# arielgabizon/barretenberg

Measured on AMD Instinct MI355X. Metric: BN254 G1 MSM points/sec at n=2^20 (Fr NTT elems/sec in 'ntt'), higher is better.
Workload: dtype u32x9 (256-bit Montgomery, 29-bit limbs)

## Files before the change

barretenberg_amd/csrc/capi.hip:

```cpp
#include <hip/hip_runtime.h>

#include <algorithm>
#include <mutex>
#include <optional>
#include <stdarg.h>
#include <stdio.h>
#include <stdlib.h>
#include <string.h>
#include <time.h>
#include <atomic>
#include <condition_variable>
#include <exception>
#include <functional>
#include <thread>
#include <unordered_map>
#include <vector>

#include "bbgpu_internal.h"
#include "host_g1.hpp"
#include "host_g2.hpp"
#include "host_small.hpp"
#include "host_fallback.hpp"
#include "host_copy_pool.hpp"
#include "host_pairing.hpp"
#include "host_srs_check.hpp"
#include "host_srs_update.hpp"
#include "host_plonk_verify.hpp"
#include "multi_plan.hpp"
#include "poly.h"

namespace bbgpu {

static thread_local char g_err[512] = "";
void set_error(const char* fmt, ...)
{
    va_list ap;
    va_start(ap, fmt);
    vsnprintf(g_err, sizeof(g_err), fmt, ap);
    va_end(ap);
}

namespace {
enum FaultKind { F_ALLOC = 0, F_H2D = 1, F_D2H = 2, F_LAUNCH = 3, F_KINDS = 4 };
struct FaultState {
    std::mutex mu;
    std::atomic<int> armed_kind{ -1 };
    uint64_t fail_at = 0;
    std::atomic<uint64_t> calls[F_KINDS] = {};
    std::atomic<uint64_t> fired{ 0 }, absorbed{ 0 };
    std::unordered_map<void*, size_t> live;
    uint64_t live_bytes = 0;
    bool env_read = false;
};
FaultState& fault()
{
    static FaultState* f = new FaultState();
    return *f;
}
int fault_parse(const char* spec, int* kind, uint64_t* at)
{
    static const char* names[F_KINDS] = { "alloc", "h2d", "d2h", "launch" };
    if (!spec || !*spec) { *kind = -1; return 0; }
    for (int k = 0; k < F_KINDS; k++) {
        const size_t len = strlen(names[k]);
        if (!strncmp(spec, names[k], len) && spec[len] == ':') {
            char* end = nullptr;
            *at = strtoull(spec + len + 1, &end, 0);
            if (end == spec + len + 1 || *end) return -1;
            *kind = k;
            return 0;
        }
    }
    return -1;
}
int fault_set(const char* spec)
{
    FaultState& F = fault();
    int kind = -1;
    uint64_t at = 0;
    if (fault_parse(spec, &kind, &at)) return -1;
    std::lock_guard<std::mutex> lk(F.mu);
    F.env_read = true;
    for (auto& c : F.calls) c.store(0);
    F.fired.store(0);
    F.absorbed.store(0);
    F.fail_at = at;
    F.armed_kind.store(kind);
    return 0;
}
bool fault_hit(FaultKind kind)
{
    FaultState& F = fault();
    if (!F.env_read) {
        std::lock_guard<std::mutex> lk(F.mu);
        if (!F.env_read) {
            F.env_read = true;
            int k = -1;
            uint64_t at = 0;
            const char* e = getenv("BBGPU_FAIL_AT");
            if (e && fault_parse(e, &k, &at) == 0 && k >= 0) {
                F.fail_at = at;
                F.armed_kind.store(k);
            } else if (e && *e) {
                fprintf(stderr, "bbgpu: BBGPU_FAIL_AT=%s not understood (alloc:k | h2d:k | d2h:k | launch:k)\n", e);
            }
        }
    }
    const uint64_t n = F.calls[kind].fetch_add(1);
    if (F.armed_kind.load(std::memory_order_relaxed) != (int)kind) return false;
    std::lock_guard<std::mutex> lk(F.mu);
    if (F.armed_kind.load() != (int)kind || n != F.fail_at) return false;
// ... 28 lines not shown
        auto it = F.live.find(p);
        if (it != F.live.end()) {
            F.live_bytes -= it->second;
            F.live.erase(it);
        }
    }
    return hipFree(p);
}
hipError_t h2d_async(void* dst, const void* src, size_t bytes, hipStream_t st)
{
    if (fault_hit(F_H2D)) {
        set_error("hipMemcpyAsync(host to device, %zu bytes) -> %s [injected by BBGPU_FAIL_AT]", bytes, hipGetErrorString(hipErrorInvalidValue));
        return hipErrorInvalidValue;
    }
    return hipMemcpyAsync(dst, src, bytes, hipMemcpyHostToDevice, st);
}
hipError_t d2h_async(void* dst, const void* src, size_t bytes, hipStream_t st)
{
    if (fault_hit(F_D2H)) {
        set_error("hipMemcpyAsync(device to host, %zu bytes) -> %s [injected by BBGPU_FAIL_AT]", bytes, hipGetErrorString(hipErrorInvalidValue));
        return hipErrorInvalidValue;
    }
    return hipMemcpyAsync(dst, src, bytes, hipMemcpyDeviceToHost, st);
}
hipError_t launch_check()
{
    const hipError_t e = hipGetLastError();
    if (e != hipSuccess) return e;
    if (fault_hit(F_LAUNCH)) {
        set_error("kernel launch -> %s [injected by BBGPU_FAIL_AT]", hipGetErrorString(hipErrorLaunchFailure));
        return hipErrorLaunchFailure;
    }
    return hipSuccess;
}
void fault_absorbed() { fault().absorbed.fetch_add(1); }

namespace {

struct SrsEntry {
    const uint64_t* host_ptr;
    size_t n;
    uint32_t* d_srs;
    bool live;
    struct TabSeg {
        size_t first = 0, n = 0;
        uint32_t* d_tab = nullptr;
        uint32_t* d_tab_alloc = nullptr;
    };
    std::vector<TabSeg> segs;
    bool has_tab() const { return !segs.empty(); }
    int tab_c = 0, tab_W = 0, tab_wb = 0, tab_we = 0;
    std::vector<uint64_t> row_hash;
    bool auto_registered = false;
    uint64_t last_use = 0;
    size_t bytes = 0;
    bool handle_exposed = false;
    uint64_t check_phase = 0;
    bool stale_for_host = false;
    bool validate_full = false;
};

inline uint64_t hash_row(const uint64_t* row8)
{
    static const uint64_t M[8] = { 0x9e3779b97f4a7c15ULL, 0xbf58476d1ce4e5b9ULL, 0x94d049bb133111ebULL, 0xd6e8feb86659fd93ULL,
                                   0xca5a826395121157ULL, 0xff51afd7ed558ccdULL, 0xc4ceb9fe1a85ec53ULL, 0x2545f4914f6cdd1dULL };
    uint64_t h = 0;
    for (int i = 0; i < 8; i++) h += (row8[i] ^ M[(i + 3) & 7]) * M[i];
    h ^= h >> 31;
    return h * 0x9e3779b97f4a7c15ULL;
}

struct Context {
    bool ready = false;
    int device = 0;
    hipStream_t stream = nullptr;
    std::vector<SrsEntry> srs;
    static constexpr int NSLOT = 8;
    MsmSlot slot[NSLOT];
    int next_slot = 0;
    uint64_t* d_stage = nullptr;
    size_t stage_cap = 0;
    uint64_t* d_stage2 = nullptr;
    size_t stage2_cap = 0;
    uint64_t* d_scratch = nullptr;
    size_t scratch_cap = 0;
    uint64_t* d_small_tab = nullptr;
    size_t small_tab_cap = 0;
    uint64_t* d_srs_check = nullptr;
    size_t srs_check_cap = 0;
    uint64_t* d_verify = nullptr;
    size_t verify_cap = 0;
    int timing = 0;
    bool precompute = true;
    uint64_t use_clock = 0;
    size_t srs_cache_cap = (size_t)16 << 30;
    bool srs_validate_full = false;
    int host_msm_max = 24;
    int host_ntt_max = 16;
    bool host_env_read = false;
    int share_rank = 0, share_world = 1;
    int point_world = 1;
    hipEvent_t helper_dep[NSLOT] = {};
    hipEvent_t shared_done = nullptr;
    hipStream_t shared_last = nullptr;
    bool shared_used = false;
    poly::Scratch poly_scratch;
    uint64_t* d_poly_tmp = nullptr;
    size_t poly_tmp_cap = 0;
    MsmTiming last;
    static constexpr size_t HOST_CHUNK = (size_t)1 << 20;
    static constexpr int HOST_RING = 8;
    size_t host_chunk = HOST_CHUNK;
    void* h_stage[HOST_RING] = {};
    hipEvent_t h_stage_free[HOST_RING] = {};
    unsigned h_stage_next = 0;
    size_t host_stage_max = (size_t)8 << 20;
    bool stage_env_read = false;
    host::CopyPool copy_pool;
    AccRing acc_ring;
    size_t slice_of_n = 0;
    std::recursive_mutex own_mu;
};

std::recursive_mutex g_mu;
Context g_ctxs[BBGPU_MAX_CONTEXTS];
int g_num_ctx = 1;
thread_local int t_ctx = 0;
inline Context& ctx() { return g_ctxs[t_ctx]; }
inline std::recursive_mutex& ctx_lock() { return t_ctx == 0 ? g_mu : ctx().own_mu; }

#define CHK(x)                                                                                                         \
    do {                                                                                                               \
        hipError_t e_ = (x);                                                                                           \
        if (e_ != hipSuccess) {                                                                                        \
            set_error("%s:%d %s -> %s", __FILE__, __LINE__, #x, hipGetErrorString(e_));                                \
            return BBGPU_ERR_HIP;                                                                                      \
        }                                                                                                              \
    } while (0)

void read_host_env()
{
    if (!ctx().host_env_read) {
        ctx().host_env_read = true;
        if (const char* e = getenv("BBGPU_HOST_MSM_MAX")) ctx().host_msm_max = atoi(e);
        if (const char* e = getenv("BBGPU_HOST_NTT_MAX")) ctx().host_ntt_max = std::min(64, atoi(e));
    }
    if (ctx().stage_env_read) return;
    ctx().stage_env_read = true;
    if (const char* e = getenv("BBGPU_STAGE_MAX_BYTES")) ctx().host_stage_max = (size_t)strtoull(e, nullptr, 0);
    if (const char* e = getenv("BBGPU_STAGE_CHUNK_BYTES")) ctx().host_chunk = std::min(Context::HOST_CHUNK, std::max((size_t)64 << 10, (size_t)strtoull(e, nullptr, 0)));
}

int hip_device_count()
{
    static const int cnt = [] { int c = 0; return hipGetDeviceCount(&c) == hipSuccess ? c : 0; }();
    return cnt;
}

int ensure_init()
{
    std::lock_guard<std::recursive_mutex> lk(ctx_lock());
    if (ctx().ready) {
        static thread_local int bound_device = -1;
        if (bound_device != ctx().device) {
            CHK(hipSetDevice(ctx().device));
            bound_device = ctx().device;
        }
        return BBGPU_OK;
    }
    (void)setenv("GPU_MAX_HW_QUEUES", "16", 0);
    if (hip_device_count() == 0) {
        set_error("no HIP device available: the GPU entry points of libbbgpu have no CPU fallback");
        return BBGPU_ERR_HIP;
    }
    CHK(hipSetDevice(ctx().device));
    CHK(hipStreamCreateWithFlags(&ctx().stream, hipStreamNonBlocking));
    for (auto& sl : ctx().slot) {
        if (!sl.stream) CHK(hipStreamCreateWithFlags(&sl.stream, hipStreamNonBlocking));
        sl.acc_ring = &ctx().acc_ring;
    }
    CHK(hipEventCreateWithFlags(&ctx().shared_done, hipEventDisableTiming));
    ctx().shared_used = false;
    if (const char* e = getenv("BBGPU_SRS_CACHE_BYTES")) ctx().srs_cache_cap = (size_t)strtoull(e, nullptr, 0);
    if (const char* e = getenv("BBGPU_SRS_VALIDATE")) ctx().srs_validate_full = !strcmp(e, "full");
    ctx().ready = true;
    return BBGPU_OK;
}

int shared_begin(hipStream_t st)
{
    if (ctx().shared_used && ctx().shared_last != st) CHK(hipStreamWaitEvent(st, ctx().shared_done, 0));
    return BBGPU_OK;
}
int shared_end(hipStream_t st)
{
    CHK(hipEventRecord(ctx().shared_done, st));
    ctx().shared_last = st;
    ctx().shared_used = true;
    return BBGPU_OK;
}

int grow(uint64_t** buf, size_t* cap, size_t bytes)
{
    if (bytes <= *cap) return BBGPU_OK;
    if (*buf) (void)dev_free(*buf);
    *buf = nullptr;
    *cap = 0;
    CHK(dev_malloc((void**)buf, bytes));
    *cap = bytes;
    return BBGPU_OK;
}

}


int bind_calling_thread()
{
    return ensure_init();
}
static int host_stage_ensure()
{
    for (int k = 0; k < Context::HOST_RING; k++)
        if (!ctx().h_stage[k]) {
            CHK(hipHostMalloc(&ctx().h_stage[k], Context::HOST_CHUNK, hipHostMallocDefault));
            CHK(hipEventCreateWithFlags(&ctx().h_stage_free[k], hipEventDisableTiming));
        }
    return BBGPU_OK;
}
int host_to_device(void* d_dst, const void* h_src, size_t bytes, hipStream_t st)
{
    std::lock_guard<std::recursive_mutex> lk(ctx_lock());
    read_host_env();
    if (bytes == 0) return BBGPU_OK;
    if (bytes > ctx().host_stage_max) {
        CHK(h2d_async(d_dst, h_src, bytes, st));
        return BBGPU_OK;
    }
    if (int rc = host_stage_ensure()) return rc;
    const size_t CH = ctx().host_chunk;
    for (size_t off = 0; off < bytes; off += CH) {
        const size_t len = std::min(CH, bytes - off);
        const int k = (int)(ctx().h_stage_next++ % Context::HOST_RING);
        CHK(hipEventSynchronize(ctx().h_stage_free[k]));
        ctx().copy_pool.copy(ctx().h_stage[k], (const char*)h_src + off, len);
        CHK(h2d_async((char*)d_dst + off, ctx().h_stage[k], len, st));
        CHK(hipEventRecord(ctx().h_stage_free[k], st));
    }
    return BBGPU_OK;
}
int device_to_host_sync(void* h_dst, const void* d_src, size_t bytes, hipStream_t st, bool* touched)
{
    std::lock_guard<std::recursive_mutex> lk(ctx_lock());
    read_host_env();
    if (touched) *touched = false;
    if (bytes > ctx().host_stage_max) {
        CHK(d2h_async(h_dst, d_src, bytes, st));
        if (touched) *touched = true;
        CHK(hipStreamSynchronize(st));
        return BBGPU_OK;
    }
    if (int rc = host_stage_ensure()) return rc;
    const size_t CH = ctx().host_chunk;
    const size_t chunks = (bytes + CH - 1) / CH;
// ... 335 lines not shown
    const size_t stride = n / 14, phase = (size_t)((e.check_phase++ * 0x9e3779b97f4a7c15ULL) % stride);
    for (size_t k = 0; k < 14; k++)
        if (!same(phase + k * stride)) return false;
    return true;
}

bool contents_match_full(const SrsEntry& e, size_t off, const uint64_t* points, size_t n)
{
    if (e.row_hash.size() != e.n) return false;
    struct Job { const uint64_t* p; const uint64_t* h; std::atomic<int> bad; } job{ points, e.row_hash.data() + off, { 0 } };
    ctx().copy_pool.for_range(n, (size_t)1 << 14, [](void* c, size_t lo, size_t hi) {
        Job* j = static_cast<Job*>(c);
        uint64_t diff = 0;
        for (size_t i = lo; i < hi; i++) diff |= hash_row(j->p + i * 16) ^ j->h[i];
        if (diff) j->bad.store(1);
    }, &job);
    return job.bad.load() == 0;
}

struct FullCheckJob {
    const uint64_t* p = nullptr;
    const uint64_t* h = nullptr;
    std::atomic<int> bad{ 0 };
    bool posted = false;
};
void full_check_post(FullCheckJob& job, const SrsEntry& e, size_t off, const uint64_t* points, size_t n)
{
    job.p = points;
    job.h = e.row_hash.data() + off;
    job.bad.store(e.row_hash.size() != e.n ? 1 : 0);
    job.posted = true;
    if (job.bad.load()) return;
    ctx().copy_pool.post_range(n, [](void* c, size_t lo, size_t hi) {
        FullCheckJob* j = static_cast<FullCheckJob*>(c);
        uint64_t diff = 0;
        for (size_t i = lo; i < hi; i++) diff |= hash_row(j->p + i * 16) ^ j->h[i];
        if (diff) j->bad.store(1);
    }, &job);
}
bool full_check_join(FullCheckJob& job)
{
    ctx().copy_pool.join();
    job.posted = false;
    return job.bad.load() == 0;
}

int find_srs(const uint64_t* points, size_t n, size_t* offset, bool* deferred_full = nullptr)
{
    if (deferred_full) *deferred_full = false;
    for (size_t k = ctx().srs.size(); k-- > 0;) {
        SrsEntry& e = ctx().srs[k];
        if (!e.live || !e.host_ptr || e.stale_for_host) continue;
        const uint8_t* b = (const uint8_t*)e.host_ptr;
        const uint8_t* p = (const uint8_t*)points;
        if (p < b || p >= b + e.n * 128) continue;
        const size_t d = (size_t)(p - b);
        if (d % 128) continue;
        if (d / 128 + n > e.n) continue;
        if (!contents_match(e, d / 128, points, n) || (e.validate_full && !deferred_full && !contents_match_full(e, d / 128, points, n))) {
            if (trace_srs()) fprintf(stderr, "bbgpu srs: contents of %p (+%zu rows, n=%zu) differ from the resident copy\n", (const void*)e.host_ptr, d / 128, n);
            if (e.auto_registered) free_entry(e);
            else if (e.validate_full) e.stale_for_host = true;
            continue;
        }
        if (deferred_full) *deferred_full = e.validate_full;
        e.last_use = ++ctx().use_clock;
        *offset = d / 128;
        return (int)k;
    }
    return -1;
}

void srs_mark_stale(int idx)
{
    SrsEntry& e = ctx().srs[idx];
    if (trace_srs()) fprintf(stderr, "bbgpu srs: full check: contents of %p differ from the resident copy\n", (const void*)e.host_ptr);
    if (e.auto_registered) free_entry(e);
    else e.stale_for_host = true;
}

double now_ms() { timespec ts; clock_gettime(CLOCK_MONOTONIC, &ts); return ts.tv_sec * 1e3 + ts.tv_nsec * 1e-6; }

size_t largest_piece(const PointPiece* pc, int np) { size_t m = 0; for (int k = 0; k < np; k++) m = std::max(m, pc[k].len); return m; }
size_t collected_before(size_t p, int slots) { return p - std::min(p, (size_t)std::max(slots, 1) - 1); }
template <class Done> struct HostMsmPipeline {
    int sl[2] = { -1, -1 }, ns = 0;
    Done done;
    double ms_push = 0, ms_wait = 0;

    explicit HostMsmPipeline(Done d) : done(std::move(d)) {}
    HostMsmPipeline(const HostMsmPipeline&) = delete;
    ~HostMsmPipeline()
    {
        if (bg.posted) (void)full_check_join(bg);
        drain();
    }
    int open()
    {
        if (int rc = ensure_init()) return rc;
        if ((ns = free_slots(sl, 2)) == 0) {
            set_error("all %d MSM slots are in flight: call bbgpu_msm_g1_wait first", Context::NSLOT);
            return BBGPU_ERR_STATE;
        }
        reserve.emplace(sl, ns);
        return BBGPU_OK;
    }
    hipStream_t first_stream() const { return ctx().slot[sl[0]].stream; }
    int make_room() { return collected < collected_before(issued, ns) ? collect() : BBGPU_OK; }
    int push(const SrsEntry& e, size_t off, const uint64_t* scalars, size_t len, size_t stage_bytes, size_t tag, MsmTiming* timing)
    {
        if (int rc = make_room()) return rc;
        const size_t w = issued % (size_t)ns;
        MsmSlot& S = ctx().slot[sl[w]];
        const double t0 = tr ? now_ms() : 0;
        int rc = grow(stage[w], cap[w], stage_bytes);
        if (rc == BBGPU_OK) rc = host_to_device(*stage[w], scalars, len * 32, S.stream);
        if (rc == BBGPU_OK) rc = issue_ticket(sl[w], e, off, stage[w], 1, len, 0, entry_windows(e, len), S.stream);
        if (rc) { drain(); return rc; }
        if (tr) ms_push += now_ms() - t0;
        fl[w] = InFlight{ tag, timing };
        issued++;
        return BBGPU_OK;
    }
    void check_in_full(int idx, size_t off, const uint64_t* points, size_t n, bool background)
    {
        for (const auto& c : checks)
            if (c.idx == idx && c.off == off && c.n == n) return;
        if (background && checks.empty()) full_check_post(bg, ctx().srs[idx], off, points, n);
        checks.push_back(Check{ idx, off, points, n });
    }
    int finish(bool* stale)
    {
        for (size_t k = 0; k < checks.size(); k++) {
            const Check& c = checks[k];
            const bool same = (k == 0 && bg.posted) ? full_check_join(bg) : !ctx().srs[c.idx].live || contents_match_full(ctx().srs[c.idx], c.off, c.points, c.n);
            if (!same) {
                srs_mark_stale(c.idx);
                *stale = true;
            }
        }
        if (*stale) {
            drain();
            return BBGPU_OK;
        }
        while (collected < issued)
            if (int rc = collect()) return rc;
        return BBGPU_OK;
    }

private:
    struct InFlight { size_t tag; MsmTiming* timing; } fl[2] = {};
    size_t issued = 0, collected = 0;
    uint64_t** stage[2] = { &ctx().d_stage, &ctx().d_stage2 };
    size_t* cap[2] = { &ctx().stage_cap, &ctx().stage2_cap };
    std::optional<SlotReservation> reserve;
    struct Check { int idx; size_t off; const uint64_t* points; size_t n; };
    std::vector<Check> checks;
    FullCheckJob bg;
    const bool tr = trace_srs();

    int collect()
    {
        const size_t w = collected++ % (size_t)ns;
        const double t0 = tr ? now_ms() : 0;
        host::Xyzz sum;
        if (int rc = finish_ticket(sl[w], &sum, fl[w].timing)) { drain(); return rc; }
        done(fl[w].tag, sum);
        if (tr) ms_wait += now_ms() - t0;
        return BBGPU_OK;
    }
    void drain()
    {
        drain_tickets(sl, ns);
        collected = issued;
    }
};

template <class Once> int rerun_if_stale(Once once)
{
    bool stale = false;
    int rc = once(&stale);
    if (stale) rc = once(&stale);
    return rc;
}

int log2_exact(size_t n)
{
    if (n == 0 || (n & (n - 1))) return -1;
    int l = 0;
    while (((size_t)1 << l) < n) l++;
    return l;
}

int msm_host_ptrs_once(const uint64_t* scalars, const uint64_t* points, size_t n, host::Xyzz* out, bool plain, bool* stale);
int msm_host_ptrs_sum(const uint64_t* scalars, const uint64_t* points, size_t n, host::Xyzz* out, bool plain = false)
{
    return rerun_if_stale([&](bool* stale) { return msm_host_ptrs_once(scalars, points, n, out, plain, stale); });
}
int msm_host_ptrs(const uint64_t* scalars, const uint64_t* points, size_t n, uint64_t out[12], bool plain = false)
{
    host::Xyzz res;
    const int rc = msm_host_ptrs_sum(scalars, points, n, &res, plain);
    if (rc == BBGPU_OK) host::g1_to_normalised(res, out);
    return rc;
}
int msm_host_ptrs_once(const uint64_t* scalars, const uint64_t* points, size_t n, host::Xyzz* out, bool plain, bool* stale)
{
    *stale = false;
    if (n == 0) {
        *out = host::g1_infinity();
        return BBGPU_OK;
    }
    if (!scalars || !points) {
        set_error("null scalars/points");
        return BBGPU_ERR_ARG;
    }
    size_t off = 0;
    bool full_check = false;
    int idx = plain ? -1 : find_srs(points, n, &off, &full_check);
    read_host_env();
    if (idx < 0 && n <= (size_t)ctx().host_msm_max) {
        *out = host::msm_small(scalars, points, n, plain ? 8 : 16);
        return BBGPU_OK;
    }
    host::Xyzz res = host::g1_infinity();
    HostMsmPipeline P([&res](size_t, const host::Xyzz& part) { res = host::g1_add(res, part); });
    if (int rc = P.open()) return rc;
    if (full_check) P.check_in_full(idx, off, points, n, n * 32 > ctx().host_stage_max);
    SrsEntry transient{};
    const bool is_transient = idx < 0 && (plain || n < AUTO_REGISTER_MIN_POINTS);
    const bool tr = trace_srs();
    const double q0 = tr ? now_ms() : 0;
    const bool small_once = is_transient && n < AUTO_REGISTER_MIN_POINTS;
    if (idx < 0) {
        uint32_t* d = nullptr;
        int rc = BBGPU_OK;
        if (small_once) {
            if ((rc = grow(&ctx().d_small_tab, &ctx().small_tab_cap, AUTO_REGISTER_MIN_POINTS * (128 + 64))) != BBGPU_OK) return rc;
            uint32_t* d_raw = (uint32_t*)ctx().d_small_tab;
            d = d_raw + AUTO_REGISTER_MIN_POINTS * 32;
            rc = srs_upload_into(points, n, d_raw, d, P.first_stream(), plain ? 64 : 128);
        } else {
            rc = srs_upload(points, n, &d, ctx().stream, plain ? 64 : 128);
        }
        if (rc) return rc;
        if (is_transient) {
            transient.host_ptr = points;
            transient.n = n;
            transient.d_srs = d;
            transient.live = true;
        } else if ((idx = add_srs(points, n, d, true)) < 0) {
            return idx;
        }
        off = 0;
    }
    const SrsEntry& e = is_transient ? transient : ctx().srs[idx];
    static const size_t split_env = [] { const char* v = getenv("BBGPU_HOST_MSM_SPLIT"); return v ? (size_t)std::min(MAX_POINT_PIECES, std::max(1, atoi(v))) : (size_t)0; }();
    PointPiece pc[MAX_POINT_PIECES];
    int np = split_pieces(e, off, n, pc, MAX_POINT_PIECES);
    if (np < 0) return BBGPU_ERR_SIZE;
    if (np == 1) {
        const size_t parts = P.ns < 2 ? 1 : (split_env ? split_env : (n >= ((size_t)1 << 19) ? 2 : 1));
        const size_t base = parts == 2 ? ((n * 3 / 8) & ~(size_t)7) : n / parts;
        np = 0;
        for (size_t k = 0; k < parts; k++) {
            const size_t o = k * base, len = (k + 1 == parts) ? n - o : base;
            if (len) pc[np++] = PointPiece{ nullptr, 0, o, len };
        }
    }
    const size_t stage_bytes = largest_piece(pc, np) * 32;
    const double q1 = tr ? now_ms() : 0;
    int rc = BBGPU_OK;
    for (int k = 0; k < np && rc == BBGPU_OK; k++)
        rc = P.push(e, off + pc[k].first, scalars + pc[k].first * 4, pc[k].len, stage_bytes, (size_t)k, k + 1 == np ? &ctx().last : nullptr);
    if (rc == BBGPU_OK) rc = P.finish(stale);
    const double q3 = tr ? now_ms() : 0;
    if (is_transient && !small_once) (void)dev_free(transient.d_srs);
    if (rc || *stale) return rc;
    *out = res;
    if (tr) fprintf(stderr, "bbgpu msm n=%zu: table %.3f, upload + issue %.3f, wait + host sums %.3f, free %.3f ms\n", n, q1 - q0, P.ms_push, P.ms_wait, now_ms() - q3);
    return BBGPU_OK;
}

struct MultiWorker {
    std::mutex mu;
    std::condition_variable cv;
    std::function<int()> job;
    bool busy = false, stop = false;
    int rc = BBGPU_OK;
    std::exception_ptr ex;
    char err[sizeof(g_err)] = "";
    std::thread th;
    explicit MultiWorker(int k) { th = std::thread([this, k] { loop(k); }); }
    void loop(int k)
    {
        t_ctx = k;
        std::unique_lock<std::mutex> lk(mu);
        for (;;) {
            cv.wait(lk, [&] { return stop || job; });
            if (!job) return;
            std::function<int()> fn = std::move(job);
            job = nullptr;
            lk.unlock();
            g_err[0] = 0;
            int r = BBGPU_ERR_STATE;
            std::exception_ptr e;
            try {
                r = fn();
            } catch (...) {
                e = std::current_exception();
            }
            lk.lock();
            rc = r;
            ex = e;
            memcpy(err, g_err, sizeof(err));
            busy = false;
            cv.notify_all();
        }
    }
    void post(std::function<int()> fn)
    {
        std::lock_guard<std::mutex> lk(mu);
        job = std::move(fn);
        busy = true;
        cv.notify_all();
    }
    int wait(char* err_out, std::exception_ptr* ex_out = nullptr)
    {
        std::unique_lock<std::mutex> lk(mu);
        cv.wait(lk, [&] { return !busy; });
        memcpy(err_out, err, sizeof(err));
        if (ex_out) *ex_out = ex;
        ex = nullptr;
        return rc;
    }
    void join()
    {
        {
            std::lock_guard<std::mutex> lk(mu);
            stop = true;
            cv.notify_all();
        }
        th.join();
    }
};
MultiWorker* g_workers[BBGPU_MAX_CONTEXTS] = {};

int run_on_contexts(int m, const std::function<int(int)>& fn)
{
    for (int k = 1; k < m; k++) g_workers[k]->post([&fn, k] { return fn(k); });
    std::exception_ptr thrown;
    int rc = BBGPU_ERR_STATE;
    try {
        rc = fn(0);
    } catch (...) {
        thrown = std::current_exception();
    }
    int bad = rc ? 0 : -1;
    char text[sizeof(g_err)];
    memcpy(text, g_err, sizeof(text));
    for (int k = 1; k < m; k++) {
        char e[sizeof(g_err)];
        std::exception_ptr ex;
        const int r = g_workers[k]->wait(e, &ex);
        if (ex && !thrown) thrown = ex;
        if (r != BBGPU_OK && bad < 0) {
            rc = r;
            bad = k;
            memcpy(text, e, sizeof(text));
        }
    }
    if (thrown) std::rethrow_exception(thrown);
    if (bad >= 0) {
        text[sizeof(text) - 1] = 0;
        set_error("context %d (device %d): %s", bad, g_ctxs[bad].device, text);
    }
    return rc;
}

void release_context(bool primary)
{
    Context& C = ctx();
    if (!C.ready) return;
    if (primary) plonk_release_all_locked();
    for (int k = 0; k < Context::NSLOT; k++)
        if (C.slot[k].pending && !C.slot[k].is_helper) drain_ticket(k);
    for (auto& ev : C.helper_dep) {
        if (ev) (void)hipEventDestroy(ev);
        ev = nullptr;
    }
    (void)hipStreamSynchronize(C.stream);
    for (auto& sl : C.slot)
        if (sl.stream) (void)hipStreamSynchronize(sl.stream);
    (void)hipDeviceSynchronize();
    host_stage_release();
    C.poly_scratch.release();
    if (C.d_poly_tmp) (void)dev_free(C.d_poly_tmp);
    C.d_poly_tmp = nullptr;
    C.poly_tmp_cap = 0;
    for (auto& e : C.srs) {
        if (e.live && e.d_srs) (void)dev_free(e.d_srs);
        if (e.live)
            for (auto& sg : e.segs)
                if (sg.d_tab_alloc) (void)dev_free(sg.d_tab_alloc);
    }
    C.srs.clear();
    for (auto& sl : C.slot) sl.release();
    C.acc_ring.release();
    if (C.d_stage) (void)dev_free(C.d_stage);
    if (C.d_stage2) (void)dev_free(C.d_stage2);
    C.d_stage2 = nullptr;
    C.stage2_cap = 0;
    if (C.d_scratch) (void)dev_free(C.d_scratch);
    C.d_stage = C.d_scratch = nullptr;
    C.stage_cap = C.scratch_cap = 0;
    if (C.d_small_tab) (void)dev_free(C.d_small_tab);
    C.d_small_tab = nullptr;
    C.small_tab_cap = 0;
    if (C.d_srs_check) (void)dev_free(C.d_srs_check);
    C.d_srs_check = nullptr;
    C.srs_check_cap = 0;
    if (C.d_verify) (void)dev_free(C.d_verify);
    C.d_verify = nullptr;
    C.verify_cap = 0;
    if (primary) ntt_release_tables();
    if (C.shared_done) (void)hipEventDestroy(C.shared_done);
    C.shared_done = nullptr;
    C.shared_used = false;
    (void)hipStreamDestroy(C.stream);
    C.stream = nullptr;
    C.ready = false;
}

void shutdown_locked()
{
    for (int k = g_num_ctx - 1; k >= 1; k--) {
        if (!g_workers[k]) continue;
        char e[sizeof(g_err)];
        g_workers[k]->post([] { release_context(false); return BBGPU_OK; });
        (void)g_workers[k]->wait(e);
        g_workers[k]->join();
        delete g_workers[k];
        g_workers[k] = nullptr;
    }
    g_num_ctx = 1;
    release_context(true);
}

void add_context_memory(const Context& C, bool primary, bbgpu_memory_info* out)
{
    for (const auto& e : C.srs) {
        if (!e.live) continue;
        const uint64_t pts = (uint64_t)e.n * 64, tab = e.bytes > pts ? e.bytes - pts : 0;
        out->srs_points_bytes += pts;
        out->srs_table_bytes += tab;
        if (e.auto_registered) out->srs_auto_bytes += e.bytes;
    }
    out->srs_cache_cap_bytes += C.srs_cache_cap;
    if (primary) {
        size_t cap = 0;
        int sets = 0;
        out->ntt_table_bytes += ntt_table_bytes(&cap, &sets);
        out->ntt_table_cap_bytes += cap;
        out->ntt_table_sets += (uint64_t)sets;
    }
    for (const auto& sl : C.slot) {
        out->msm_workspace_bytes += sl.ws.cap;
        if (sl.ws.h_out) out->pinned_host_bytes += (uint64_t)MSM_HOUT_GROUPS * 64 * 128;
    }
    out->staging_bytes += C.stage_cap + C.stage2_cap + C.scratch_cap + C.poly_tmp_cap + C.poly_scratch.cap + C.small_tab_cap + C.srs_check_cap + C.verify_cap;
    if (primary) out->staging_bytes += plonk_lane_bytes();
    for (int k = 0; k < Context::HOST_RING; k++)
        if (C.h_stage[k]) out->pinned_host_bytes += Context::HOST_CHUNK;
}

}
}

using namespace bbgpu;

#pragma GCC visibility push(default)
extern "C" {

const char* bbgpu_version(void) { return "bbgpu 0.1 (gfx950)"; }
const char* bbgpu_last_error(void) { return g_err; }

int bbgpu_device_count(void)
{
    int cnt = 0;
    if (hipGetDeviceCount(&cnt) != hipSuccess) return 0;
    return cnt;
}

int bbgpu_init(int device)
{
    std::lock_guard<std::recursive_mutex> lk(g_mu);
    if (ctx().ready && ctx().device == device) return BBGPU_OK;
    if (ctx().ready) {
        set_error("already bound to %d context(s), the first on device %d: bbgpu_shutdown() first", g_num_ctx, ctx().device);
        return BBGPU_ERR_STATE;
    }
    ctx().device = device;
    return ensure_init();
}

int bbgpu_init_devices(const int* devices, int count)
{
    if (!devices || count < 1 || count > BBGPU_MAX_CONTEXTS) {
        set_error("bbgpu_init_devices: %s (1 to %d contexts)", devices ? "bad context count" : "null device list", BBGPU_MAX_CONTEXTS);
        return BBGPU_ERR_ARG;
    }
    for (int k = 0; k < count; k++)
        if (devices[k] < 0) {
            set_error("bbgpu_init_devices: negative device %d for context %d", devices[k], k);
            return BBGPU_ERR_ARG;
        }
    std::lock_guard<std::mutex> lkp(plonk_mutex());
    std::lock_guard<std::recursive_mutex> lk(g_mu);
    if (g_ctxs[0].ready) {
        bool same = g_num_ctx == count;
        for (int k = 0; same && k < count; k++) same = g_ctxs[k].device == devices[k];
        if (same) return BBGPU_OK;
        set_error("already bound to %d context(s), the first on device %d: bbgpu_shutdown() first", g_num_ctx, g_ctxs[0].device);
        return BBGPU_ERR_STATE;
    }
    const int cnt = hip_device_count();
    if (cnt == 0) {
        set_error("no HIP device available: the GPU entry points of libbbgpu have no CPU fallback");
        return BBGPU_ERR_HIP;
    }
    for (int k = 0; k < count; k++)
        if (devices[k] >= cnt) {
            set_error("bbgpu_init_devices: device %d of context %d, the machine has %d", devices[k], k, cnt);
            return BBGPU_ERR_ARG;
        }
    g_ctxs[0].device = devices[0];
    if (int rc = ensure_init()) return rc;
    for (int k = 1; k < count; k++) {
        g_ctxs[k].device = devices[k];
        g_workers[k] = new MultiWorker(k);
        g_num_ctx = k + 1;
        g_workers[k]->post([] { return ensure_init(); });
        char e[sizeof(g_err)];
        if (int rc = g_workers[k]->wait(e)) {
            shutdown_locked();
            e[sizeof(e) - 1] = 0;
            set_error("context %d (device %d): %s", k, devices[k], e);
            return rc;
        }
    }
    return BBGPU_OK;
}

// ... 843 lines not shown
{
    return msm_num_windows(msm_choose_c(n ? n : 1));
}
int bbgpu_srs_num_windows(int srs_handle, size_t n)
{
    std::lock_guard<std::recursive_mutex> lk(g_mu);
    if (srs_handle < 0 || srs_handle >= (int)ctx().srs.size() || !ctx().srs[srs_handle].live) return BBGPU_ERR_ARG;
    return entry_windows(ctx().srs[srs_handle], n);
}
void bbgpu_set_table_share(int rank, int world)
{
    std::lock_guard<std::recursive_mutex> lk(g_mu);
    if (world < 1 || rank < 0 || rank >= world) { rank = 0; world = 1; }
    ctx().share_rank = rank;
    ctx().share_world = world;
}

void bbgpu_set_point_share(int world)
{
    std::lock_guard<std::recursive_mutex> lk(g_mu);
    ctx().point_world = world >= 1 && world <= 1024 ? world : 1;
}

void bbgpu_set_precompute(int enabled)
{
    std::lock_guard<std::recursive_mutex> lk(g_mu);
    for (auto& C : g_ctxs) C.precompute = enabled != 0;
}

int bbgpu_msm_g1(const uint64_t* scalars, const uint64_t* points_endo_table, size_t n, uint64_t out[12])
{
    std::lock_guard<std::recursive_mutex> lk(g_mu);
    multi::Slice sl[BBGPU_MAX_CONTEXTS];
    const int m = multi::plan_slices(n, g_num_ctx, sl);
    if (m == 1) return msm_host_ptrs(scalars, points_endo_table, n, out);
    if (!scalars || !points_endo_table) {
        set_error("null scalars/points");
        return BBGPU_ERR_ARG;
    }
    host::Xyzz part[BBGPU_MAX_CONTEXTS];
    const int rc = run_on_contexts(m, [&](int k) {
        ctx().slice_of_n = n;
        const int r = msm_host_ptrs_sum(scalars + 4 * sl[k].first, points_endo_table + 16 * sl[k].first, sl[k].len, &part[k]);
        ctx().slice_of_n = 0;
        return r;
    });
    if (rc) return rc;
    host::Xyzz acc = part[0];
    for (int k = 1; k < m; k++) acc = host::g1_add(acc, part[k]);
    host::g1_to_normalised(acc, out);
    return BBGPU_OK;
}

int bbgpu_msm_g1_plain(const uint64_t* scalars, const uint64_t* points, size_t n, uint64_t out[12])
{
    std::lock_guard<std::recursive_mutex> lk(g_mu);
    return msm_host_ptrs(scalars, points, n, out, true);
}

void bbgpu_set_host_thresholds(int msm_max_points, int ntt_max_elements)
{
    std::lock_guard<std::recursive_mutex> lk(g_mu);
    for (auto& C : g_ctxs) {
        C.host_env_read = true;
        C.host_msm_max = msm_max_points < 0 ? 0 : msm_max_points;
        C.host_ntt_max = ntt_max_elements < 0 ? 0 : std::min(64, ntt_max_elements);
    }
}

static int batch_equal_sizes(const bbgpu_msm_job* jobs, size_t num_jobs)
{
    for (size_t i = 1; i < num_jobs; i++)
        if (jobs[i].num_elements != jobs[0].num_elements) {
            set_error("batched_scalar_multiplications err: each scalar mul must be same size.");
            return BBGPU_ERR_ARG;
        }
    return BBGPU_OK;
}
static bool batch_job_by_job(size_t n) { return n == 0 || n <= (size_t)ctx().host_msm_max; }
struct NullJob { size_t done; bool numbered; };
static NullJob batch_null_job(size_t n, size_t i, int slots)
{
    if (batch_job_by_job(n)) return NullJob{ i, false };
    return NullJob{ collected_before(i, slots), slots >= 2 };
}
static int null_job_error(const NullJob& nj, size_t i)
{
    set_error(nj.numbered ? "null scalars/points in job %zu" : "null scalars/points", i);
    return BBGPU_ERR_ARG;
}
static int msm_g1_batch_once(bbgpu_msm_job* jobs, size_t num_jobs, bool* stale, host::Xyzz* sums);
static int msm_g1_batch_run(bbgpu_msm_job* jobs, size_t num_jobs, host::Xyzz* sums)
{
    return rerun_if_stale([&](bool* stale) { return msm_g1_batch_once(jobs, num_jobs, stale, sums); });
}
static int msm_g1_batch_split(bbgpu_msm_job* jobs, size_t num_jobs, const multi::Slice* sl, int m)
{
    if (num_jobs == 0) return BBGPU_OK;
    const size_t n = jobs[0].num_elements;
    std::vector<bbgpu_msm_job> local((size_t)m * num_jobs);
    std::vector<host::Xyzz> part((size_t)m * num_jobs);
    for (int k = 0; k < m; k++)
        for (size_t i = 0; i < num_jobs; i++) {
            bbgpu_msm_job& J = local[(size_t)k * num_jobs + i];
            J = jobs[i];
            J.points = jobs[i].points + 16 * sl[k].first;
            J.scalars = jobs[i].scalars + 4 * sl[k].first;
            J.num_elements = sl[k].len;
        }
    const int rc = run_on_contexts(m, [&](int k) {
        ctx().slice_of_n = n;
        const int r = msm_g1_batch_run(&local[(size_t)k * num_jobs], num_jobs, &part[(size_t)k * num_jobs]);
        ctx().slice_of_n = 0;
        return r;
    });
    if (rc) return rc;
    for (size_t i = 0; i < num_jobs; i++) {
        host::Xyzz acc = part[i];
        for (int k = 1; k < m; k++) acc = host::g1_add(acc, part[(size_t)k * num_jobs + i]);
        host::g1_to_normalised(acc, jobs[i].output);
    }
    return BBGPU_OK;
}
int bbgpu_msm_g1_batch(bbgpu_msm_job* jobs, size_t num_jobs)
{
    std::lock_guard<std::recursive_mutex> lk(g_mu);
    multi::Slice sl[BBGPU_MAX_CONTEXTS];
    const int m = (num_jobs && jobs) ? multi::plan_slices(jobs[0].num_elements, g_num_ctx, sl) : 1;
    if (m == 1) return msm_g1_batch_run(jobs, num_jobs, nullptr);
    if (int rc = batch_equal_sizes(jobs, num_jobs)) return rc;
    const size_t n = jobs[0].num_elements;
    for (size_t i = 0; i < num_jobs; i++)
        if (!jobs[i].scalars || !jobs[i].points) {
            read_host_env();
            int fs[2];
            const NullJob nj = batch_null_job(n, i, free_slots(fs, 2));
            if (int rc = msm_g1_batch_split(jobs, nj.done, sl, m)) return rc;
            return null_job_error(nj, i);
        }
    return msm_g1_batch_split(jobs, num_jobs, sl, m);
}
static int msm_g1_batch_once(bbgpu_msm_job* jobs, size_t num_jobs, bool* stale, host::Xyzz* sums)
{
    *stale = false;
    int rc = BBGPU_OK;
    if (num_jobs == 0) return BBGPU_OK;
    if (!jobs) return BBGPU_ERR_ARG;
    if ((rc = batch_equal_sizes(jobs, num_jobs)) != BBGPU_OK) return rc;
    const size_t n = jobs[0].num_elements;
    read_host_env();
    if (batch_job_by_job(n)) {
        for (size_t i = 0; i < num_jobs; i++) {
            rc = sums ? msm_host_ptrs_sum(jobs[i].scalars, jobs[i].points, jobs[i].num_elements, &sums[i])
                      : msm_host_ptrs(jobs[i].scalars, jobs[i].points, jobs[i].num_elements, jobs[i].output);
            if (rc) return rc;
        }
        return BBGPU_OK;
    }
    auto null_job = [&](size_t i) { return !jobs[i].scalars || !jobs[i].points; };
    int fs[2];
    if (null_job(0)) return null_job_error(batch_null_job(n, 0, free_slots(fs, 2)), 0);
    host::Xyzz acc = host::g1_infinity();
    HostMsmPipeline P([&](size_t tag, const host::Xyzz& part) {
        acc = host::g1_add(acc, part);
        if (!(tag & 1)) return;
        if (sums) sums[tag >> 1] = acc;
        else host::g1_to_normalised(acc, jobs[tag >> 1].output);
        acc = host::g1_infinity();
    });
    if ((rc = P.open()) != BBGPU_OK) return rc;
    const bool tr = trace_srs();
    for (size_t i = 0; i < num_jobs; i++) {
        const double push0 = P.ms_push, wait0 = P.ms_wait;
        if ((rc = P.make_room()) != BBGPU_OK) return rc;
        if (null_job(i)) return null_job_error(batch_null_job(n, i, P.ns), i);
        const double q1 = tr ? now_ms() : 0;
        size_t off = 0;
        bool full_check = false;
        int idx = find_srs(jobs[i].points, n, &off, &full_check);
        if (idx < 0) {
            uint32_t* d = nullptr;
            if ((rc = srs_upload(jobs[i].points, n, &d, ctx().stream)) != BBGPU_OK) return rc;
            if ((idx = add_srs(jobs[i].points, n, d, true)) < 0) return idx;
        }
        if (full_check) P.check_in_full(idx, off, jobs[i].points, n, false);
        const double q2 = tr ? now_ms() : 0;
        PointPiece pc[MAX_POINT_PIECES];
        const int np = split_pieces(ctx().srs[idx], off, n, pc, MAX_POINT_PIECES);
        if (np < 0) return BBGPU_ERR_SIZE;
        const size_t stage_bytes = largest_piece(pc, np) * 32;
        for (int k = 0; k < np; k++)
            if ((rc = P.push(ctx().srs[idx], off + pc[k].first, jobs[i].scalars + pc[k].first * 4, pc[k].len, stage_bytes, i * 2 + (k + 1 == np), nullptr)) != BBGPU_OK) return rc;
        if (tr) fprintf(stderr, "bbgpu batch: job %zu (%d ranges) srs %.3f, upload + issue %.3f, wait for earlier jobs %.3f ms\n", i, np, q2 - q1, P.ms_push - push0, P.ms_wait - wait0);
    }
    const double wait0 = P.ms_wait;
    rc = P.finish(stale);
    if (tr) fprintf(stderr, "bbgpu batch: last wait %.3f ms\n", P.ms_wait - wait0);
    return rc;
}

static int ticket_srs(int srs_handle, const SrsEntry** e)
{
    if (int rc = ensure_init()) return rc;
    if (srs_handle < 0 || srs_handle >= (int)ctx().srs.size() || !ctx().srs[srs_handle].live) {
        set_error("unknown SRS handle %d", srs_handle);
        return BBGPU_ERR_ARG;
    }
    *e = &ctx().srs[srs_handle];
    return BBGPU_OK;
}
static int share_ticket_srs(int srs_handle, size_t offset, const uint64_t* d_scalars, size_t n, const char* kind, const SrsEntry** ep)
{
    if (int rc = ticket_srs(srs_handle, ep)) return rc;
    const SrsEntry& e = **ep;
    if (offset + n > e.n || !d_scalars || n == 0) {
        set_error("MSM range [%zu, %zu) outside the registered table of %zu points", offset, offset + n, e.n);
        return BBGPU_ERR_ARG;
    }
    if (e.segs.size() != 1) {
        set_error(e.has_tab() ? "%s-range shares need ONE table segment: this SRS of %zu points keeps %zu (split it by point range instead)"
                              : "%s-range shares need the pre-shifted window tables (one shared bucket set): this table has none", kind, e.n, e.segs.size());
        return BBGPU_ERR_STATE;
    }
    return BBGPU_OK;
}
static int begin_ticket(void* hip_stream, int* t, hipStream_t* st)
{
    if ((*t = pick_slot()) < 0) return BBGPU_ERR_STATE;
    MsmSlot& S = ctx().slot[*t];
    *st = hip_stream ? (hipStream_t)hip_stream : S.stream;
    S.helper = -1;
    S.append = false;
    S.throughput = others_pending(&S);
    return BBGPU_OK;
}
static int commit_ticket(int t)
{
    if (t < 2) ctx().next_slot = t ^ 1;
    return t;
}

int bbgpu_msm_g1_device(int srs_handle, size_t offset, const uint64_t* d_scalars, size_t n, int window_begin, int window_end,
                        uint64_t out[12], void* hip_stream)
{
    int ticket = bbgpu_msm_g1_device_async(srs_handle, offset, d_scalars, n, window_begin, window_end, hip_stream);
    if (ticket < 0) return ticket;
    return bbgpu_msm_g1_wait(ticket, out);
}

int bbgpu_msm_g1_device_async(int srs_handle, size_t offset, const uint64_t* d_scalars, size_t n, int window_begin, int window_end,
                              void* hip_stream)
{
    std::lock_guard<std::recursive_mutex> lk(g_mu);
    const SrsEntry* ep = nullptr;
    if (int rc = ticket_srs(srs_handle, &ep)) return rc;
    const SrsEntry& e = *ep;
    if (offset + n > e.n || (!d_scalars && n)) {
        set_error("MSM range [%zu, %zu) outside the registered table of %zu points", offset, offset + n, e.n);
        return BBGPU_ERR_ARG;
    }
    int t;
    hipStream_t st;
    if (int rc = begin_ticket(hip_stream, &t, &st)) return rc;
    const int rc = issue_ticket(t, e, offset, &d_scalars, 1, n, window_begin, window_end, st);
    if (rc == BBGPU_ERR_ARG) set_error("bad window range [%d, %d)", window_begin, window_end);
    return rc ? rc : commit_ticket(t);
}

namespace {
struct VerifierHandle {
    host::VerifyKey K;
    VerifyDeviceKey D;
    uint64_t shared_rows[host::VERIFY_MAX_SHARED * 8];
// ... 270 lines not shown
```

Baseline: 948.7 million.

## Upload next MSM scalar range on a separate stream while slots are busy

Adds a third device staging buffer, a dedicated upload stream and per-buffer events. When both MSM slots are still busy, the next range's scalars are copied host-to-device on the upload stream before waiting to collect an earlier result, and the slot stream then waits on that copy's event. The aim is to hide scalar upload latency behind the previous range's computation rather than serialising copy after collect. This costs more staging memory and extra cross-stream synchronisation.

```diff
diff --git a/barretenberg_amd/csrc/capi.hip b/barretenberg_amd/csrc/capi.hip
--- a/barretenberg_amd/csrc/capi.hip
+++ b/barretenberg_amd/csrc/capi.hip
@@ -27,6 +27,7 @@
 #include "host_srs_update.hpp"
 #include "host_plonk_verify.hpp"
 #include "multi_plan.hpp"
+#include "host_msm_plan.hpp"
 #include "poly.h"
 
 namespace bbgpu {
@@ -221,6 +222,10 @@
     size_t stage_cap = 0;
     uint64_t* d_stage2 = nullptr;
     size_t stage2_cap = 0;
+    uint64_t* d_stage3 = nullptr;
+    size_t stage3_cap = 0;
+    hipStream_t upload_stream = nullptr;
+    hipEvent_t staged[hostplan::STAGE_BUFFERS] = {};
     uint64_t* d_scratch = nullptr;
     size_t scratch_cap = 0;
     uint64_t* d_small_tab = nullptr;
@@ -318,6 +323,7 @@
         if (!sl.stream) CHK(hipStreamCreateWithFlags(&sl.stream, hipStreamNonBlocking));
         sl.acc_ring = &ctx().acc_ring;
     }
+    CHK(hipStreamCreateWithFlags(&ctx().upload_stream, hipStreamNonBlocking));
     CHK(hipEventCreateWithFlags(&ctx().shared_done, hipEventDisableTiming));
     ctx().shared_used = false;
     if (const char* e = getenv("BBGPU_SRS_CACHE_BYTES")) ctx().srs_cache_cap = (size_t)strtoull(e, nullptr, 0);
@@ -819,9 +825,18 @@
 double now_ms() { timespec ts; clock_gettime(CLOCK_MONOTONIC, &ts); return ts.tv_sec * 1e3 + ts.tv_nsec * 1e-6; }
 
 size_t largest_piece(const PointPiece* pc, int np) { size_t m = 0; for (int k = 0; k < np; k++) m = std::max(m, pc[k].len); return m; }
-size_t collected_before(size_t p, int slots) { return p - std::min(p, (size_t)std::max(slots, 1) - 1); }
+int plan_call_ranges(const SrsEntry& e, size_t off, size_t n, int slots, int first_eighths, bool one_range, PointPiece* pc)
+{
+    static const size_t split_env = [] { const char* v = getenv("BBGPU_HOST_MSM_SPLIT"); return v ? (size_t)std::min(MAX_POINT_PIECES, std::max(1, atoi(v))) : (size_t)0; }();
+    int np = split_pieces(e, off, n, pc, MAX_POINT_PIECES);
+    if (np != 1 || one_range) return np;
+    hostplan::Range r[MAX_POINT_PIECES];
+    np = hostplan::plan_ranges(n, slots, split_env, first_eighths, r, MAX_POINT_PIECES);
+    for (int k = 0; k < np; k++) pc[k] = PointPiece{ nullptr, 0, r[k].first, r[k].len };
+    return np;
+}
 template <class Done> struct HostMsmPipeline {
-    int sl[2] = { -1, -1 }, ns = 0;
+    int sl[hostplan::MAX_SLOTS] = { -1, -1 }, ns = 0;
     Done done;
     double ms_push = 0, ms_wait = 0;
 
@@ -839,24 +854,39 @@
             set_error("all %d MSM slots are in flight: call bbgpu_msm_g1_wait first", Context::NSLOT);
             return BBGPU_ERR_STATE;
         }
+        rot.slots = ns;
         reserve.emplace(sl, ns);
         return BBGPU_OK;
     }
     hipStream_t first_stream() const { return ctx().slot[sl[0]].stream; }
-    int make_room() { return collected < collected_before(issued, ns) ? collect() : BBGPU_OK; }
+    int make_room()
+    {
+        while (rot.to_collect())
+            if (int rc = collect()) return rc;
+        return BBGPU_OK;
+    }
     int push(const SrsEntry& e, size_t off, const uint64_t* scalars, size_t len, size_t stage_bytes, size_t tag, MsmTiming* timing)
     {
-        if (int rc = make_room()) return rc;
-        const size_t w = issued % (size_t)ns;
+        const hostplan::Rotation::Step at = rot.stage();
+        const int w = at.slot, b = at.buffer;
         MsmSlot& S = ctx().slot[sl[w]];
+        const bool ahead = rot.slot_busy();
         const double t0 = tr ? now_ms() : 0;
-        int rc = grow(stage[w], cap[w], stage_bytes);
-        if (rc == BBGPU_OK) rc = host_to_device(*stage[w], scalars, len * 32, S.stream);
-        if (rc == BBGPU_OK) rc = issue_ticket(sl[w], e, off, stage[w], 1, len, 0, entry_windows(e, len), S.stream);
+        int rc = grow(stage[b], cap[b], stage_bytes);
+        if (rc == BBGPU_OK) rc = host_to_device(*stage[b], scalars, len * 32, ahead ? ctx().upload_stream : S.stream);
+        if (rc == BBGPU_OK && ahead) rc = staged_event(b);
+        went_ahead = went_ahead || ahead;
+        if (tr) ms_push += now_ms() - t0;
+        if (rc == BBGPU_OK) rc = make_room();
+        else drain();
+        if (rc) return rc;
+        const double t1 = tr ? now_ms() : 0;
+        if (ahead) rc = hip_rc(hipStreamWaitEvent(S.stream, ctx().staged[b], 0), "hipStreamWaitEvent");
+        if (rc == BBGPU_OK) rc = issue_ticket(sl[w], e, off, stage[b], 1, len, 0, entry_windows(e, len), S.stream);
         if (rc) { drain(); return rc; }
-        if (tr) ms_push += now_ms() - t0;
+        if (tr) ms_push += now_ms() - t1;
         fl[w] = InFlight{ tag, timing };
-        issued++;
+        rot.issue();
         return BBGPU_OK;
     }
     void check_in_full(int idx, size_t off, const uint64_t* points, size_t n, bool background)
@@ -880,25 +910,38 @@
             drain();
             return BBGPU_OK;
         }
-        while (collected < issued)
+        while (rot.collected < rot.issued)
             if (int rc = collect()) return rc;
         return BBGPU_OK;
     }
 
 private:
-    struct InFlight { size_t tag; MsmTiming* timing; } fl[2] = {};
-    size_t issued = 0, collected = 0;
-    uint64_t** stage[2] = { &ctx().d_stage, &ctx().d_stage2 };
-    size_t* cap[2] = { &ctx().stage_cap, &ctx().stage2_cap };
+    struct InFlight { size_t tag; MsmTiming* timing; } fl[hostplan::MAX_SLOTS] = {};
+    hostplan::Rotation rot;
+    bool went_ahead = false;
+    uint64_t** stage[hostplan::STAGE_BUFFERS] = { &ctx().d_stage, &ctx().d_stage2, &ctx().d_stage3 };
+    size_t* cap[hostplan::STAGE_BUFFERS] = { &ctx().stage_cap, &ctx().stage2_cap, &ctx().stage3_cap };
     std::optional<SlotReservation> reserve;
     struct Check { int idx; size_t off; const uint64_t* points; size_t n; };
     std::vector<Check> checks;
     FullCheckJob bg;
     const bool tr = trace_srs();
 
+    static int hip_rc(hipError_t e, const char* what)
+    {
+        if (e == hipSuccess) return BBGPU_OK;
+        set_error("%s -> %s", what, hipGetErrorString(e));
+        return BBGPU_ERR_HIP;
+    }
+    int staged_event(int b)
+    {
+        if (!ctx().staged[b])
+            if (int rc = hip_rc(hipEventCreateWithFlags(&ctx().staged[b], hipEventDisableTiming), "hipEventCreateWithFlags")) return rc;
+        return hip_rc(hipEventRecord(ctx().staged[b], ctx().upload_stream), "hipEventRecord");
+    }
     int collect()
     {
-        const size_t w = collected++ % (size_t)ns;
+        const int w = rot.collect();
         const double t0 = tr ? now_ms() : 0;
         host::Xyzz sum;
         if (int rc = finish_ticket(sl[w], &sum, fl[w].timing)) { drain(); return rc; }
@@ -909,7 +952,9 @@
     void drain()
     {
         drain_tickets(sl, ns);
-        collected = issued;
+        if (went_ahead) (void)hipStreamSynchronize(ctx().upload_stream);
+        went_ahead = false;
+        rot.drain();
     }
 };
 
@@ -992,19 +1037,9 @@
         off = 0;
     }
     const SrsEntry& e = is_transient ? transient : ctx().srs[idx];
-    static const size_t split_env = [] { const char* v = getenv("BBGPU_HOST_MSM_SPLIT"); return v ? (size_t)std::min(MAX_POINT_PIECES, std::max(1, atoi(v))) : (size_t)0; }();
     PointPiece pc[MAX_POINT_PIECES];
-    int np = split_pieces(e, off, n, pc, MAX_POINT_PIECES);
+    const int np = plan_call_ranges(e, off, n, P.ns, hostplan::SINGLE_FIRST_EIGHTHS, small_once, pc);
     if (np < 0) return BBGPU_ERR_SIZE;
-    if (np == 1) {
-        const size_t parts = P.ns < 2 ? 1 : (split_env ? split_env : (n >= ((size_t)1 << 19) ? 2 : 1));
-        const size_t base = parts == 2 ? ((n * 3 / 8) & ~(size_t)7) : n / parts;
-        np = 0;
-        for (size_t k = 0; k < parts; k++) {
-            const size_t o = k * base, len = (k + 1 == parts) ? n - o : base;
-            if (len) pc[np++] = PointPiece{ nullptr, 0, o, len };
-        }
-    }
     const size_t stage_bytes = largest_piece(pc, np) * 32;
     const double q1 = tr ? now_ms() : 0;
     int rc = BBGPU_OK;
@@ -1127,6 +1162,7 @@
         ev = nullptr;
     }
     (void)hipStreamSynchronize(C.stream);
+    if (C.upload_stream) (void)hipStreamSynchronize(C.upload_stream);
     for (auto& sl : C.slot)
         if (sl.stream) (void)hipStreamSynchronize(sl.stream);
     (void)hipDeviceSynchronize();
@@ -1146,8 +1182,15 @@
     C.acc_ring.release();
     if (C.d_stage) (void)dev_free(C.d_stage);
     if (C.d_stage2) (void)dev_free(C.d_stage2);
-    C.d_stage2 = nullptr;
-    C.stage2_cap = 0;
+    if (C.d_stage3) (void)dev_free(C.d_stage3);
+    C.d_stage2 = C.d_stage3 = nullptr;
+    C.stage2_cap = C.stage3_cap = 0;
+    for (auto& ev : C.staged) {
+        if (ev) (void)hipEventDestroy(ev);
+        ev = nullptr;
+    }
+    if (C.upload_stream) (void)hipStreamDestroy(C.upload_stream);
+    C.upload_stream = nullptr;
     if (C.d_scratch) (void)dev_free(C.d_scratch);
     C.d_stage = C.d_scratch = nullptr;
     C.stage_cap = C.scratch_cap = 0;
@@ -1205,7 +1248,7 @@
         out->msm_workspace_bytes += sl.ws.cap;
         if (sl.ws.h_out) out->pinned_host_bytes += (uint64_t)MSM_HOUT_GROUPS * 64 * 128;
     }
-    out->staging_bytes += C.stage_cap + C.stage2_cap + C.scratch_cap + C.poly_tmp_cap + C.poly_scratch.cap + C.small_tab_cap + C.srs_check_cap + C.verify_cap;
+    out->staging_bytes += C.stage_cap + C.stage2_cap + C.stage3_cap + C.scratch_cap + C.poly_tmp_cap + C.poly_scratch.cap + C.small_tab_cap + C.srs_check_cap + C.verify_cap;
     if (primary) out->staging_bytes += plonk_lane_bytes();
     for (int k = 0; k < Context::HOST_RING; k++)
         if (C.h_stage[k]) out->pinned_host_bytes += Context::HOST_CHUNK;
@@ -2215,7 +2258,7 @@
 static NullJob batch_null_job(size_t n, size_t i, int slots)
 {
     if (batch_job_by_job(n)) return NullJob{ i, false };
-    return NullJob{ collected_before(i, slots), slots >= 2 };
+    return NullJob{ hostplan::collected_before_issue(i, slots), slots >= 2 };
 }
 static int null_job_error(const NullJob& nj, size_t i)
 {
@@ -2305,8 +2348,10 @@
     const bool tr = trace_srs();
     for (size_t i = 0; i < num_jobs; i++) {
         const double push0 = P.ms_push, wait0 = P.ms_wait;
-        if ((rc = P.make_room()) != BBGPU_OK) return rc;
-        if (null_job(i)) return null_job_error(batch_null_job(n, i, P.ns), i);
+        if (null_job(i)) {
+            if ((rc = P.make_room()) != BBGPU_OK) return rc;
+            return null_job_error(batch_null_job(n, i, P.ns), i);
+        }
         const double q1 = tr ? now_ms() : 0;
         size_t off = 0;
         bool full_check = false;
@@ -2319,9 +2364,14 @@
         if (full_check) P.check_in_full(idx, off, jobs[i].points, n, false);
         const double q2 = tr ? now_ms() : 0;
         PointPiece pc[MAX_POINT_PIECES];
-        const int np = split_pieces(ctx().srs[idx], off, n, pc, MAX_POINT_PIECES);
+        const int np = plan_call_ranges(ctx().srs[idx], off, n, P.ns, num_jobs > 1 ? hostplan::BATCH_FIRST_EIGHTHS : hostplan::SINGLE_FIRST_EIGHTHS, i > 0, pc);
         if (np < 0) return BBGPU_ERR_SIZE;
-        const size_t stage_bytes = largest_piece(pc, np) * 32;
+        size_t stage_points = largest_piece(pc, np);
+        if (i == 0 && num_jobs > 1) {
+            PointPiece whole[MAX_POINT_PIECES];
+            stage_points = std::max(stage_points, largest_piece(whole, std::max(0, split_pieces(ctx().srs[idx], off, n, whole, MAX_POINT_PIECES))));
+        }
+        const size_t stage_bytes = stage_points * 32;
         for (int k = 0; k < np; k++)
             if ((rc = P.push(ctx().srs[idx], off + pc[k].first, jobs[i].scalars + pc[k].first * 4, pc[k].len, stage_bytes, i * 2 + (k + 1 == np), nullptr)) != BBGPU_OK) return rc;
         if (tr) fprintf(stderr, "bbgpu batch: job %zu (%d ranges) srs %.3f, upload + issue %.3f, wait for earlier jobs %.3f ms\n", i, np, q2 - q1, P.ms_push - push0, P.ms_wait - wait0);
diff --git a/barretenberg_amd/csrc/host_msm_plan.hpp b/barretenberg_amd/csrc/host_msm_plan.hpp
--- /dev/null
+++ b/barretenberg_amd/csrc/host_msm_plan.hpp
@@ -0,0 +1,71 @@
+#pragma once
+#include <assert.h>
+#include <stddef.h>
+
+namespace bbgpu {
+namespace hostplan {
+
+constexpr int MAX_SLOTS = 2;
+constexpr int STAGE_BUFFERS = MAX_SLOTS + 1;
+constexpr size_t RANGES_MIN_POINTS = (size_t)1 << 19;
+constexpr int SINGLE_FIRST_EIGHTHS = 3;
+constexpr int BATCH_FIRST_EIGHTHS = 3;
+
+struct Range {
+    size_t first, len;
+};
+
+inline int plan_ranges(size_t n, int free_slots, size_t split, int first_eighths, Range* out, int cap)
+{
+    size_t parts = free_slots < 2 ? 1 : (split ? split : (n >= RANGES_MIN_POINTS ? 2 : 1));
+    if (parts > (size_t)cap) parts = (size_t)cap;
+    const size_t base = parts == 2 ? ((n * (size_t)first_eighths / 8) & ~(size_t)7) : n / parts;
+    int cnt = 0;
+    for (size_t k = 0; k < parts; k++) {
+        const size_t o = k * base, len = (k + 1 == parts) ? n - o : base;
+        if (len) out[cnt++] = Range{ o, len };
+    }
+    return cnt;
+}
+
+inline size_t collected_before_issue(size_t p, int slots)
+{
+    const size_t keep = (size_t)(slots < 1 ? 1 : slots) - 1;
+    return p - (p < keep ? p : keep);
+}
+inline size_t collected_before_stage(size_t p)
+{
+    const size_t keep = (size_t)STAGE_BUFFERS - 1;
+    return p - (p < keep ? p : keep);
+}
+
+struct Rotation {
+    int slots = 1;
+    size_t issued = 0, collected = 0;
+
+    struct Step {
+        int slot, buffer;
+    };
+    Step stage() const
+    {
+        assert(slots >= 1 && slots <= MAX_SLOTS);
+        assert(collected >= collected_before_stage(issued));
+        return Step{ (int)(issued % (size_t)slots), (int)(issued % (size_t)STAGE_BUFFERS) };
+    }
+    size_t to_collect() const
+    {
+        const size_t want = collected_before_issue(issued, slots);
+        return want > collected ? want - collected : 0;
+    }
+    bool slot_busy() const { return issued - collected >= (size_t)slots; }
+    int collect() { return (int)(collected++ % (size_t)slots); }
+    void issue()
+    {
+        assert(to_collect() == 0);
+        issued++;
+    }
+    void drain() { collected = issued; }
+};
+
+}
+}
```

Result: no change. 948.3 million (-0.0%).
